# benmcclusky/Residual-TD3-Robot-Navigation

Measured on AMD Instinct MI355X. Metric: env-steps/sec at 65 536 parallel envs (full residual-TD3 update), higher is better.
Workload: dtype f32-accurate MLP: fp16x2 split (22-bit operands) on fp16 MFMA, f32 accumulate; f32 edge layers / losses / Adam; fp64 env state; 1 GPU; config3: 65536 envs + residual-TD3 (2x256 MLPs); envs_per_gpu=65536, envs_per_group=1024, hidden=256, layers=2, batch=32768, rank_batch=32768, parallelism=independent-env-blocks x1

## Files before the change

### residual-td3-robot-navigation_amd/csrc/learner_kernels.hip

```cpp
#include "mlp_common.h"

namespace {

struct WgradArgs {
    MlpDev net[2];
    int64_t M;
    const float* in;
    int ld_in, in_col;
    const float* acts[2];
    const float* dz[2];
    const float* dy[2];
    int ld_dy;
    const uint16_t* masks[2];
    float* slabs[2];
    int splits;
    int tk;
    int TT;
    int tn;
    int TN;
    int n_hid;
    int fact;
    int64_t per_split;
    int64_t per_wave;
    int64_t skew;
};

#ifdef NAV_WGRAD_TRACE
__device__ unsigned long long g_wgrad_trace[2][4][8][8];
#define WG_MARK(kid, k)                                                                        \
    do {                                                                                       \
        const int b_ = blockIdx.x == 0 ? 0 : blockIdx.x == 1 ? 1 : blockIdx.x == 128 ? 2         \
                       : blockIdx.x == 255 ? 3 : -1;                                           \
        if (b_ >= 0 && (threadIdx.x & 63) == 0)                                                \
            g_wgrad_trace[kid][b_][threadIdx.x >> 6][k] = __builtin_readcyclecounter();         \
    } while (0)
#else
#define WG_MARK(kid, k) \
    do {                \
    } while (0)
#endif

constexpr int WG_WAVES = 8;
#ifndef NAV_WG_SKEW_FACT
#define NAV_WG_SKEW_FACT 64
#endif
#ifndef NAV_WG_SKEW_OPND
#define NAV_WG_SKEW_OPND 128
#endif
constexpr int WG_TOTAL = 256;
constexpr int WG_THREADS = WG_WAVES * 64;
constexpr int WG_TILE = 64;
constexpr int WG_CHUNK = 64;
constexpr int WG_STAGE_FLOATS = WG_CHUNK * 6;
inline size_t wgrad_lds_bytes() {
    return ((size_t)WG_WAVES * WG_TILE * WG_TILE + (size_t)WG_WAVES * 2 * WG_STAGE_FLOATS) * 4;
}
__host__ __device__ inline bool wgrad_fact_ok(int hp, int n_hidden) {
    return n_hidden == 2 && hp % WG_TILE == 0;
}
struct WgradTiling {
    int tn, tk, TN, TT, jobs;
};
inline WgradTiling wgrad_tiling(int d_out, int hp, int n_hidden) {
    WgradTiling t;
    const bool f1 = wgrad_fact_ok(hp, n_hidden) && d_out == 1;
    const bool wide = f1 && hp % 256 == 0;
    t.tn = wide ? 256 : f1 && hp % 128 == 0 ? 128 : WG_TILE;
    t.tk = wide ? 32 : WG_TILE;
    t.TN = (hp + t.tn - 1) / t.tn;
    t.TT = (hp + t.tk - 1) / t.tk;
    t.jobs = (n_hidden > 1 ? n_hidden - 1 : 0) * t.TN * t.TT;
    return t;
}

template <bool PR, bool QR, bool RA_ = false>
NAV_DEV void wgrad_rows(const WgradArgs& a, int y, int L, int n0, int k0, int64_t r_lo,
                        int64_t r_hi, float* stage, f32x16 (&acc)[2][2]) {
    const MlpDev& net = a.net[y];
    const int hp = net.hp, nh = net.n_hidden, d_in = net.d_in, d_out = net.d_out;
    const int lane = threadIdx.x & 63, h = lane >> 5, l32 = lane & 31;
    const int64_t M = a.M, MH = M * hp;
    const bool nv1 = n0 + 32 < hp, kv1 = k0 + 32 < hp;
    const int cn[2] = {n0 + l32, nv1 ? n0 + 32 + l32 : n0 + l32};
    const int ck[2] = {k0 + l32, kv1 ? k0 + 32 + l32 : k0 + l32};
    float wo[2][2] = {{0.f, 0.f}, {0.f, 0.f}}, w0[2][4] = {}, b0[2] = {0.f, 0.f};
    if (PR) {
        const float* Wo = net.params + net.w_off[nh];
#pragma unroll
        for (int i = 0; i < 2; ++i) {
            wo[i][0] = Wo[cn[i]];
            wo[i][1] = d_out > 1 ? Wo[hp + cn[i]] : 0.f;
        }
    }
    if (QR) {
        const float* W0 = net.params + net.w_off[0];
        const float* bb = net.params + net.b_off[0];
#pragma unroll
        for (int j = 0; j < 2; ++j) {
#pragma unroll
            for (int k = 0; k < 4; ++k) w0[j][k] = k < d_in ? W0[ck[j] * d_in + k] : 0.f;
            b0[j] = bb[ck[j]];
        }
    }
    constexpr bool RA = RA_ && (PR != QR);
    constexpr int HS = WG_CHUNK / 8;
    const int NTm = hp >> 5;
// ... 67 lines not shown
            if ((!RA || s % HS == 0) && rb + 2 * s >= r_hi) break;
            if constexpr (RA) {
                if (s % HS == 0) window(s);
            }
            const int rr = 2 * s + h;
            float p[2], q[2];
            if (PR) {
                const float2 g = *reinterpret_cast<const float2*>(gs + rr * 2);
                const int sh = 16 * ((s >> 1) & 1) + 2 * (s & 1) + 4 * ((s & 15) >> 2);
#pragma unroll
                for (int i = 0; i < 2; ++i) {
                    const uint32_t bit = (mw[i][s >> 4] >> sh) & 1u;
                    p[i] = bit ? top_unit(g.x, g.y, wo[i][0], wo[i][1]) : 0.f;
                }
            } else if constexpr (RA) {
#pragma unroll
                for (int i = 0; i < 2; ++i) p[i] = ps[RA && !PR ? s % HS : 0][i];
            } else {
                const int64_t r = rb + rr;
                const bool ok = r < r_hi;
                const float* src = Psv + (ok ? r : r_lo) * hp;
#pragma unroll
                for (int i = 0; i < 2; ++i) p[i] = ok ? src[cn[i]] : 0.f;
            }
            if (QR) {
                const float4 x = *reinterpret_cast<const float4*>(xs + rr * 4);
#pragma unroll
                for (int j = 0; j < 2; ++j) q[j] = layer0_unit(x, w0[j][0], w0[j][1], w0[j][2], w0[j][3], b0[j]);
            } else if constexpr (RA) {
#pragma unroll
                for (int j = 0; j < 2; ++j) q[j] = qs[RA && !QR ? s % HS : 0][j];
            } else {
                const int64_t r = rb + rr;
                const bool ok = r < r_hi;
                const float* src = Qsv + (ok ? r : r_lo) * hp;
#pragma unroll
                for (int j = 0; j < 2; ++j) q[j] = ok ? src[ck[j]] : 0.f;
            }
            acc[0][0] = mfma(p[0], q[0], acc[0][0]);
            if (kv1) acc[0][1] = mfma(p[0], q[1], acc[0][1]);
            if (nv1) acc[1][0] = mfma(p[1], q[0], acc[1][0]);
            if (nv1 && kv1) acc[1][1] = mfma(p[1], q[1], acc[1][1]);
        }
        if (more) {
            park();
#pragma unroll
            for (int i = 0; i < 2; ++i)
#pragma unroll
                for (int t = 0; t < 2; ++t) mw[i][t] = cm[i][t] >> h;
        }
    }
}

NAV_DEV void row_maxima(const WgradArgs& a, int y, int64_t r_lo, int64_t r_hi, float (&G)[2],
                        float (&X)[4]) {
    const int lane = threadIdx.x & 63, d_in = a.net[y].d_in, d_out = a.net[y].d_out;
    float g0 = 0.f, g1 = 0.f, x0 = 0.f, x1 = 0.f, x2 = 0.f, x3 = 0.f;
    constexpr int RU = 4;
    const float* xin = a.in + a.in_col;
    const bool xv4 = d_in == 4 && (a.ld_in & 3) == 0 && ((uintptr_t)xin & 15) == 0;
    const bool xv2 = d_in == 2 && (a.ld_in & 1) == 0 && ((uintptr_t)xin & 7) == 0;
    const bool gv2 = d_out == 2 && (a.ld_dy & 1) == 0 && ((uintptr_t)a.dy[y] & 7) == 0;
    for (int64_t rb = r_lo; rb < r_hi; rb += 64 * RU) {
        float gv[RU][2], xv[RU][4];
#pragma unroll
        for (int u = 0; u < RU; ++u) {
            gv[u][0] = gv[u][1] = 0.f;
            xv[u][0] = xv[u][1] = xv[u][2] = xv[u][3] = 0.f;
            if (rb + 64 * u >= r_hi) continue;
            const int64_t r = rb + 64 * u + lane;
            if (r >= r_hi) continue;
            const float* g = a.dy[y] + r * a.ld_dy;
            const float* x = xin + r * a.ld_in;
            if (gv2) {
                const float2 v = *reinterpret_cast<const float2*>(g);
                gv[u][0] = v.x;
                gv[u][1] = v.y;
            } else {
                gv[u][0] = g[0];
                if (d_out > 1) gv[u][1] = g[1];
            }
            if (xv4) {
                const float4 v = *reinterpret_cast<const float4*>(x);
                xv[u][0] = v.x; xv[u][1] = v.y; xv[u][2] = v.z; xv[u][3] = v.w;
            } else if (xv2) {
                const float2 v = *reinterpret_cast<const float2*>(x);
                xv[u][0] = v.x; xv[u][1] = v.y;
            } else {
#pragma unroll
                for (int i = 0; i < 4; ++i)
                    if (d_in > i) xv[u][i] = x[i];
            }
        }
#pragma unroll
        for (int u = 0; u < RU; ++u) {
            g0 = fmaxf(g0, fabsf(gv[u][0]));
            g1 = fmaxf(g1, fabsf(gv[u][1]));
            x0 = fmaxf(x0, fabsf(xv[u][0]));
            x1 = fmaxf(x1, fabsf(xv[u][1]));
            x2 = fmaxf(x2, fabsf(xv[u][2]));
            x3 = fmaxf(x3, fabsf(xv[u][3]));
        }
    }
    auto su = [](float v) { return __int_as_float(__builtin_amdgcn_readfirstlane(__float_as_int(wave_max_abs(v)))); };
    G[0] = su(g0);
    G[1] = su(g1);
    X[0] = su(x0);
    X[1] = su(x1);
    X[2] = su(x2);
    X[3] = su(x3);
}

NAV_DEV float h0_bound(const float (&X)[4], float wa, float wb, float bias) {
    const int h = (threadIdx.x & 63) >> 5;
    const float part = (h ? X[1] : X[0]) * fabsf(wa) + (h ? X[3] : X[2]) * fabsf(wb) + fabsf(bias);
    return part + __shfl_xor(part, 32, 64);
}

NAV_DEV int cap_exp_finite(int e, float m) {
    if (!(m > 0.f)) return e;
    int E;
    (void)frexpf(m, &E);
    return min(e, 126 - E);
}

NAV_DEV void wgrad_rows_mfma(const WgradArgs& a, int y, int n0, int k0, int64_t r_lo,
                             int64_t r_hi, f32x16 (&acc)[2][2]) {
    const MlpDev& net = a.net[y];
    const int hp = net.hp, nh = net.n_hidden, d_in = net.d_in, d_out = net.d_out;
    const int lane = threadIdx.x & 63, h = lane >> 5, l32 = lane & 31;
    const int64_t M = a.M;
    const int NTm = hp >> 5;
    float wob[2], w0b[2][2], bob[2];
    {
        const float* Wo = net.params + net.w_off[nh];
        const float* W0 = net.params + net.w_off[0];
        const float* bb = net.params + net.b_off[0];
#pragma unroll
        for (int i = 0; i < 2; ++i) {
            wob[i] = h < d_out ? Wo[h * hp + n0 + 32 * i + l32] : 0.f;
            const int c = k0 + 32 * i + l32;
            w0b[i][0] = h < d_in ? W0[c * d_in + h] : 0.f;
            w0b[i][1] = 2 + h < d_in ? W0[c * d_in + 2 + h] : 0.f;
            bob[i] = h == 0 ? bb[c] : 0.f;
        }
    }
    if (r_lo >= r_hi) return;
    const uint16_t* mk = a.masks[y] + (size_t)(nh - 1) * mask_rowtiles(M) * NTm * 64 +
                         (size_t)(n0 >> 5) * 64 + lane;
    const size_t mstride = (size_t)NTm * 64;
    const float* dyp = a.dy[y];
    const int ld_dy = a.ld_dy, ld_in = a.ld_in;
    const float* xin = a.in + a.in_col;
    const int gk = h < d_out ? h : 0, xk0 = h < d_in ? h : 0, xk1 = 2 + h < d_in ? 2 + h : 0;
    struct Raw {
        float g, x0, x1;
        uint32_t m0, m1;
    };
    const float* gp = dyp + (r_lo + l32) * ld_dy + gk;
    const float* xp = xin + (r_lo + l32) * ld_in;
    const uint16_t* mp = mk + (size_t)(r_lo >> 5) * mstride;
    const int64_t gstep = 32 * (int64_t)ld_dy, xstep = 32 * (int64_t)ld_in;
    int64_t rl = r_lo;
    auto load = [&](int64_t) {
        Raw v;
        if (rl + 32 <= r_hi) {
            v.g = *gp;
            v.x0 = xp[xk0];
            v.x1 = xp[xk1];
            v.m0 = mp[0];
            v.m1 = mp[64];
        } else {
            const bool ok = rl + l32 < r_hi;
            const float* g = ok ? gp : dyp + r_lo * ld_dy + gk;
            const float* x = ok ? xp : xin + r_lo * ld_in;
            v.g = *g;
            v.x0 = x[xk0];
            v.x1 = x[xk1];
            v.m0 = mp[0];
            v.m1 = mp[64];
        }
        gp += gstep;
        xp += xstep;
        mp += mstride;
        rl += 32;
        return v;
    };
    float bc[2];
    const bool x23 = d_in > 2;
    auto issue = [&](int64_t rt, const Raw& v, f32x16 (&P)[2], f32x16 (&Q)[2]) {
        const bool ok = rt + l32 < r_hi && h < d_out;
        const float g = ok ? v.g : 0.f;
        const float x0 = h < d_in ? v.x0 : 0.f, x1 = 2 + h < d_in ? v.x1 : 0.f;
        const f32x16 zero = {};
#pragma unroll
        for (int i = 0; i < 2; ++i) {
            P[i] = mfma(g, wob[i], zero);
            f32x16 b;
#pragma unroll
            for (int e = 0; e < 16; ++e) b[e] = bc[i];
            Q[i] = mfma(x0, w0b[i][0], b);
        }
        if (x23) {
#pragma unroll
            for (int i = 0; i < 2; ++i) Q[i] = mfma(x1, w0b[i][1], Q[i]);
        }
    };
    auto finish = [&](const Raw& v, f32x16 (&P)[2], f32x16 (&Q)[2]) {
#pragma unroll
        for (int e = 0; e < 16; ++e) {
            P[0][e] = __int_as_float(__float_as_int(P[0][e]) & __builtin_amdgcn_sbfe((int)v.m0, e, 1));
            P[1][e] = __int_as_float(__float_as_int(P[1][e]) & __builtin_amdgcn_sbfe((int)v.m1, e, 1));
            Q[0][e] = __int_as_float(max(__float_as_int(Q[0][e]), 0));
            Q[1][e] = __int_as_float(max(__float_as_int(Q[1][e]), 0));
        }
    };
    Raw cur = load(r_lo);
    Raw nxt = cur;
    if (r_lo + 32 < r_hi) nxt = load(r_lo + 32);
    int ep[2], eq[2];
    {
        float G[2], X[4];
        WG_MARK(1, 2);
        row_maxima(a, y, r_lo, r_hi, G, X);
        WG_MARK(1, 3);
#pragma unroll
        for (int i = 0; i < 2; ++i) {
            float b = G[h] * fabsf(wob[i]);
            b += __shfl_xor(b, 32, 64);
#pragma unroll
            for (int m = 1; m < 32; m <<= 1) b = fmaxf(b, __shfl_xor(b, m, 64));
            ep[i] = pow2_exp(b);
            wob[i] = ldexpf(wob[i], ep[i]);
            float wm = fmaxf(fmaxf(fabsf(w0b[i][0]), fabsf(w0b[i][1])), fabsf(bob[i]));
            wm = fmaxf(wm, __shfl_xor(wm, 32, 64));
            eq[i] = cap_exp_finite(pow2_exp(h0_bound(X, w0b[i][0], w0b[i][1], bob[i])), wm);
            w0b[i][0] = ldexpf(w0b[i][0], eq[i]);
            w0b[i][1] = ldexpf(w0b[i][1], eq[i]);
            bob[i] = ldexpf(bob[i], eq[i]);
            bc[i] = bob[i] + __shfl_xor(bob[i], 32, 64);
        }
    }
    for (int64_t rt = r_lo; rt < r_hi; rt += 32) {
        Raw nn = nxt;
        if (rt + 64 < r_hi) nn = load(rt + 64);
        f32x16 P[2], Q[2];
        issue(rt, cur, P, Q);
        finish(cur, P, Q);
#pragma unroll
        for (int s2 = 0; s2 < 2; ++s2) {
            Split2 sp[2], sq[2];
#pragma unroll
            for (int i = 0; i < 2; ++i) {
                float vp[8], vq[8];
#pragma unroll
                for (int t = 0; t < 8; ++t) {
                    vp[t] = P[i][8 * s2 + t];
                    vq[t] = Q[i][8 * s2 + t];
                }
                sp[i] = split2_8(vp);
                sq[i] = split2_8(vq);
            }
#pragma unroll
            for (int i = 0; i < 2; ++i)
#pragma unroll
                for (int j = 0; j < 2; ++j) acc[i][j] = mfma_x3s(sp[i], sq[j], acc[i][j]);
        }
        cur = nxt;
        nxt = nn;
    }
    WG_MARK(1, 4);
#pragma unroll
    for (int i = 0; i < 2; ++i)
#pragma unroll
        for (int j = 0; j < 2; ++j)
#pragma unroll
            for (int e = 0; e < 16; ++e) acc[i][j][e] = ldexpf(acc[i][j][e], -(ep[i] + eq[j]));
}



template <int NI, int D, int KH, bool GV, bool XV>
NAV_DEV void wgrad_rows_fact(const WgradArgs& a, int y, int n0, int k0, int64_t r_lo,
                             int64_t r_hi, const char* tab, f32x16 (&out)[NI][KH]) {
    const MlpDev& net = a.net[y];
    const int hp = net.hp, d_in = net.d_in;
    const int lane = threadIdx.x & 63, h = lane >> 5, l32 = lane & 31;
    const int64_t M = a.M;
    const int NTm = hp >> 5;
    f32x16 acc[D][NI][KH];
#pragma unroll
    for (int d = 0; d < D; ++d)
#pragma unroll
        for (int i = 0; i < NI; ++i)
#pragma unroll
            for (int j = 0; j < KH; ++j)
#pragma unroll
                for (int e = 0; e < 16; ++e) acc[d][i][j][e] = 0.f;
    float w0b[KH][2], bob[KH];
    {
        const float* W0 = net.params + net.w_off[0];
        const float* bb = net.params + net.b_off[0];
#pragma unroll
        for (int j = 0; j < KH; ++j) {
            const int c = k0 + 32 * j + l32;
            w0b[j][0] = h < d_in ? W0[c * d_in + h] : 0.f;
            w0b[j][1] = 2 + h < d_in ? W0[c * d_in + 2 + h] : 0.f;
            bob[j] = h == 0 ? bb[c] : 0.f;
        }
    }
    int eh[KH], eg[D];
    float sg[D];
    float bcj[KH];
    const bool x23 = d_in > 2;
    const size_t mstride = (size_t)NTm * 64;
    const uint16_t* mp = a.masks[y] + (size_t)mask_rowtiles(M) * mstride +
                         (size_t)(n0 >> 5) * 64 + lane + (size_t)(r_lo >> 5) * mstride;
    const float* dyp = a.dy[y];
    const int ld_dy = a.ld_dy, ld_in = a.ld_in;
    const int xk0 = h < d_in ? h : 0, xk1 = 2 + h < d_in ? 2 + h : 0;
    constexpr bool MP = NI == 8;
    constexpr int NM = MP ? NI / 2 : NI;
    struct Raw {
        float x0, x1;
        uint32_t m[NM];
    };
    auto load_masks = [&](const uint16_t* m, Raw& v) {
#pragma unroll
        for (int u = 0; u < NM; ++u)
            v.m[u] = MP ? (uint32_t)m[2 * u * 64] | ((uint32_t)m[(2 * u + 1) * 64] << 16)
                        : (uint32_t)m[u * 64];
    };
    const bool xrow4 = d_in == 4 && (ld_in & 3) == 0 && (((uintptr_t)(a.in + a.in_col)) & 15) == 0;
    auto load_raw = [&](int64_t rt, Raw& v) {
        const int64_t rx = rt + l32 < r_hi ? rt + l32 : r_lo;
        const float* x = a.in + a.in_col + rx * ld_in;
        if (xrow4) {
            const float4 u = *reinterpret_cast<const float4*>(x);
            v.x0 = h ? u.y : u.x;
            v.x1 = h ? u.w : u.z;
        } else {
            v.x0 = x[xk0];
            v.x1 = x[xk1];
        }
        load_masks(mp + (size_t)((rt - r_lo) >> 5) * mstride, v);
    };
    auto tile = [&](const Raw& cur, const float (&gs)[2][D][8]) {
        const float x0 = h < d_in ? cur.x0 : 0.f, x1 = 2 + h < d_in ? cur.x1 : 0.f;
#pragma unroll
        for (int j = 0; j < KH; ++j) {
            f32x16 Z;
#pragma unroll
            for (int e = 0; e < 16; ++e) Z[e] = bcj[j];
            Z = mfma(x0, w0b[j][0], Z);
            if (x23) Z = mfma(x1, w0b[j][1], Z);
#pragma unroll
            for (int s2 = 0; s2 < 2; ++s2)
#pragma unroll
                for (int d = 0; d < D; ++d) {
                    float q[8];
#pragma unroll
                    for (int t = 0; t < 8; ++t)
                        q[t] = __int_as_float(max(__float_as_int(Z[8 * s2 + t]), 0)) * gs[s2][d][t];
                    const Split2 sq = split2_8(q);
#pragma unroll
                    for (int i = 0; i < NI; ++i) {
                        uint32_t ta = MP ? ((cur.m[i >> 1] >> (16 * (i & 1) + 8 * s2)) & 0xFFu) << 4
                                         : (s2 == 0 ? cur.m[i] << 4 : cur.m[i] >> 4) & 0xFF0u;
                        asm volatile("" : "+v"(ta));
                        const f16x8 pi = *reinterpret_cast<const f16x8*>(tab + ta);
                        acc[d][i][j] = mfma_h(pi, sq.l, acc[d][i][j]);
// ... 13 lines not shown
                const float* g = gp + (16 * s2 + 8 * qq) * ldg;
                if (GV && D == 1) {
                    const float4 u = *reinterpret_cast<const float4*>(g);
                    gs[s2][0][4 * qq] = u.x; gs[s2][0][4 * qq + 1] = u.y;
                    gs[s2][0][4 * qq + 2] = u.z; gs[s2][0][4 * qq + 3] = u.w;
                } else if (GV) {
                    const float4 u0 = *reinterpret_cast<const float4*>(g);
                    const float4 u1 = *reinterpret_cast<const float4*>(g + 4);
                    gs[s2][0][4 * qq] = u0.x; gs[s2][D - 1][4 * qq] = u0.y;
                    gs[s2][0][4 * qq + 1] = u0.z; gs[s2][D - 1][4 * qq + 1] = u0.w;
                    gs[s2][0][4 * qq + 2] = u1.x; gs[s2][D - 1][4 * qq + 2] = u1.y;
                    gs[s2][0][4 * qq + 3] = u1.z; gs[s2][D - 1][4 * qq + 3] = u1.w;
                } else {
#pragma unroll
                    for (int t = 0; t < 4; ++t)
#pragma unroll
                        for (int d = 0; d < D; ++d) gs[s2][d][4 * qq + t] = g[t * ldg + d];
                }
            }
    };
    auto scale_g = [&](float (&gs)[2][D][8]) {
        if (D == 1) return;
#pragma unroll
        for (int s2 = 0; s2 < 2; ++s2)
#pragma unroll
            for (int d = 0; d < D; ++d)
#pragma unroll
                for (int t = 0; t < 8; ++t) gs[s2][d][t] *= sg[d];
    };
    constexpr bool GPF = D == 1;
    const int64_t nfull = (r_full - r_lo) >> 5;
    const float* xq = a.in + a.in_col + (r_lo + l32) * (int64_t)ld_in;
    const uint16_t* mq = mp;
    const float* gq = dyp + (r_lo + 4 * h) * (int64_t)ldg;
    const int64_t xstep = 32 * (int64_t)ld_in, gstep = 32 * (int64_t)ldg;
    auto load_full = [&](Raw& v, float (&gs)[2][D][8]) {
        if (XV) {
            const float4 u = *reinterpret_cast<const float4*>(xq);
            v.x0 = h ? u.y : u.x;
            v.x1 = h ? u.w : u.z;
        } else {
            v.x0 = xq[xk0];
            v.x1 = xq[xk1];
        }
        load_masks(mq, v);
        if (GPF) load_g_at(gq, gs);
        xq += xstep;
        mq += mstride;
        gq += gstep;
    };
    Raw c0, c1;
    float g0[2][D][8], g1[2][D][8];
    if (nfull > 0) load_full(c0, g0);
    {
        float G[2], X[4];
        WG_MARK(0, 2);
        row_maxima(a, y, r_lo, r_hi, G, X);
        WG_MARK(0, 3);
#pragma unroll
        for (int d = 0; d < D; ++d) {
            eg[d] = pow2_exp_to(G[d], 8);
            sg[d] = D == 1 ? 1.f : ldexpf(1.f, eg[d]);
        }
#pragma unroll
        for (int j = 0; j < KH; ++j) {
            eh[j] = __builtin_amdgcn_readfirstlane(
                pow2_exp_to(wave_max_abs(h0_bound(X, w0b[j][0], w0b[j][1], bob[j])), 7));
            if (D == 1) eh[j] = min(max(eh[j] + eg[0], -126), 120);
            eh[j] = __builtin_amdgcn_readfirstlane(cap_exp_finite(
                eh[j], wave_max_abs(fmaxf(fmaxf(fabsf(w0b[j][0]), fabsf(w0b[j][1])),
                                          fabsf(bob[j])))));
            w0b[j][0] = ldexpf(w0b[j][0], eh[j]);
            w0b[j][1] = ldexpf(w0b[j][1], eh[j]);
            bob[j] = ldexpf(bob[j], eh[j]);
            bcj[j] = bob[j] + __shfl_xor(bob[j], 32, 64);
        }
        if (D == 1) eg[0] = 0;
    }
    for (int64_t t = 0; t < nfull; ++t) {
        if (t + 1 < nfull) load_full(c1, g1);
        if (!GPF) load_g_at(dyp + (r_lo + 32 * t + 4 * h) * (int64_t)ldg, g0);
        scale_g(g0);
        tile(c0, g0);
        c0 = c1;
        if (GPF) {
#pragma unroll
            for (int s2 = 0; s2 < 2; ++s2)
#pragma unroll
                for (int d = 0; d < D; ++d)
#pragma unroll
                    for (int e = 0; e < 8; ++e) g0[s2][d][e] = g1[s2][d][e];
        }
    }
    WG_MARK(0, 4);
    if (r_full < r_hi) {
        Raw cur;
        load_raw(r_full, cur);
        float gs[2][D][8];
#pragma unroll
        for (int e = 0; e < 16; ++e) {
            const int64_t r = r_full + acc_row(e, h);
#pragma unroll
            for (int d = 0; d < D; ++d) gs[e >> 3][d][e & 7] = r < r_hi ? dyp[r * ld_dy + d] * sg[d] : 0.f;
        }
        tile(cur, gs);
    }
    const float* Wo = net.params + net.w_off[net.n_hidden];
#pragma unroll
    for (int i = 0; i < NI; ++i) {
        if (NI == 8 && i > 0 && i % 2 == 0) __builtin_amdgcn_sched_barrier(0);
#pragma unroll
        for (int q = 0; q < 4; ++q) {
            const int n = n0 + 32 * i + 8 * q + 4 * h;
            float4 wv[D];
#pragma unroll
            for (int d = 0; d < D; ++d) {
                const float* w = Wo + d * hp + n;
                wv[d] = make_float4(w[0], w[1], w[2], w[3]);
            }
#pragma unroll
            for (int t = 0; t < 4; ++t) {
                const int e = 4 * q + t;
#pragma unroll
                for (int j = 0; j < KH; ++j) {
                    const float w0 = (t == 0 ? wv[0].x : t == 1 ? wv[0].y : t == 2 ? wv[0].z : wv[0].w) * 0.5f;
                    float v = w0 * ldexpf(acc[0][i][j][e], -(eh[j] + eg[0]));
                    if (D > 1) {
                        const float w1 = (t == 0 ? wv[D - 1].x : t == 1 ? wv[D - 1].y
                                          : t == 2 ? wv[D - 1].z : wv[D - 1].w) * 0.5f;
                        v = fmaf(w1, ldexpf(acc[D - 1][i][j][e], -(eh[j] + eg[D - 1])), v);
                    }
                    out[i][j][e] = v;
                }
            }
        }
    }
}

template <int NI, int KH>
NAV_DEV void wgrad_reduce_write(const WgradArgs& a, int y, int split, int L, int n0, int k0,
                                const f32x16 (&acc)[NI][KH], float* red) {
    constexpr int T = NI * 32 * 32 * KH;
    constexpr int R = (WG_WAVES * WG_TILE * WG_TILE) / T < WG_WAVES
                          ? (WG_WAVES * WG_TILE * WG_TILE) / T : WG_WAVES;
    const MlpDev& net = a.net[y];
    const int hp = net.hp;
    const int wv = wave_id(), lane = threadIdx.x & 63, h = lane >> 5, l32 = lane & 31;
    const int rot = (lane >> 2) & 3;
    float4* mine = reinterpret_cast<float4*>(red + (wv % R) * T);
#pragma unroll
    for (int round = 0; round < WG_WAVES / R; ++round) {
        if (wv / R == round) {
#pragma unroll
            for (int i = 0; i < NI; ++i)
#pragma unroll
                for (int j = 0; j < KH; ++j) {
                    float4* p = mine + ((i * KH + j) * 64 + lane) * 4;
#pragma unroll
                    for (int c = 0; c < 4; ++c) {
                        float4 v = make_float4(acc[i][j][4 * c], acc[i][j][4 * c + 1],
                                               acc[i][j][4 * c + 2], acc[i][j][4 * c + 3]);
                        if (round) {
                            const float4 o = p[c ^ rot];
                            v = make_float4(o.x + v.x, o.y + v.y, o.z + v.z, o.w + v.w);
                        }
                        p[c ^ rot] = v;
                    }
                }
        }
        __syncthreads();
    }
    float* o = a.slabs[y] + (int64_t)split * hidden_w_count(net) + (int64_t)(L - 1) * hp * hp;
// ... 4 lines not shown
#pragma unroll
        for (int w = 0; w < R; ++w) {
            const float4* p = slots + (size_t)w * (T / 4) + (b * 64 + lane) * 4;
#pragma unroll
            for (int c = 0; c < 4; ++c) {
                const float4 u = p[c ^ rot];
                if (w == 0) {
                    v[4 * c] = u.x; v[4 * c + 1] = u.y; v[4 * c + 2] = u.z; v[4 * c + 3] = u.w;
                } else {
                    v[4 * c] += u.x; v[4 * c + 1] += u.y; v[4 * c + 2] += u.z; v[4 * c + 3] += u.w;
                }
            }
        }
        const int col = k0 + 32 * j + l32;
#pragma unroll
        for (int e = 0; e < 16; ++e) {
            const int n = n0 + 32 * i + acc_row(e, h);
            if (n < hp && col < hp) o[(int64_t)n * hp + col] = v[e];
        }
    }
}

struct TileJob {
    int y, job, split, L, n0, k0;
};
NAV_DEV TileJob wgrad_job(const WgradArgs& a, int b, int total) {
    const int v = (total % 8 == 0) ? (b % 8) * (total / 8) + b / 8 : b;
    const int grp = v / a.n_hid, TT = a.TT, TN = a.TN;
    TileJob t;
    t.job = v % a.n_hid;
    t.y = grp / a.splits;
    t.split = grp % a.splits;
    t.L = t.job / (TN * TT) + 1;
    t.n0 = ((t.job % (TN * TT)) / TT) * a.tn;
    t.k0 = (t.job % TT) * a.tk;
    return t;
}

NAV_DEV void wave_rows(const WgradArgs& a, int split, int wv, int64_t skew, int64_t& r_lo,
                       int64_t& r_hi) {
    const int64_t M = a.M;
    const int64_t s_lo = (int64_t)split * a.per_split < M ? (int64_t)split * a.per_split : M;
    const int64_t s_hi = s_lo + a.per_split < M ? s_lo + a.per_split : M;
    const int64_t pa = a.per_wave + skew, pb = a.per_wave - skew;
    const int64_t off = wv < WG_WAVES / 2 ? wv * pa : (WG_WAVES / 2) * pa + (wv - WG_WAVES / 2) * pb;
    const int64_t len = wv < WG_WAVES / 2 ? pa : pb;
    r_lo = s_lo + off < s_hi ? s_lo + off : s_hi;
    r_hi = r_lo + len < s_hi ? r_lo + len : s_hi;
}

template <int NI, int D, int KH>
NAV_DEV void wgrad_tile_fact(const WgradArgs& a, const TileJob& t, float* smem, uint4* tab) {
    WG_MARK(0, 0);
    if (threadIdx.x < 256) {
        const uint32_t b = threadIdx.x;
        uint32_t w[4];
#pragma unroll
        for (int d = 0; d < 4; ++d)
            w[d] = ((b >> (2 * d)) & 1u ? 0x4000u : 0u) | ((b >> (2 * d + 1)) & 1u ? 0x40000000u : 0u);
        tab[b] = make_uint4(w[0], w[1], w[2], w[3]);
    }
    __syncthreads();
    WG_MARK(0, 1);
    int64_t r_lo, r_hi;
    wave_rows(a, t.split, wave_id(), a.skew, r_lo, r_hi);
    f32x16 out[NI][KH];
    const char* tb = reinterpret_cast<const char*>(tab);
    const bool gv = a.ld_dy == D && ((uintptr_t)a.dy[t.y] & 15) == 0;
    const bool xv = a.net[t.y].d_in == 4 && (a.ld_in & 3) == 0 &&
                    ((uintptr_t)(a.in + a.in_col) & 15) == 0;
    if (gv && xv) wgrad_rows_fact<NI, D, KH, true, true>(a, t.y, t.n0, t.k0, r_lo, r_hi, tb, out);
    else if (gv) wgrad_rows_fact<NI, D, KH, true, false>(a, t.y, t.n0, t.k0, r_lo, r_hi, tb, out);
    else if (xv) wgrad_rows_fact<NI, D, KH, false, true>(a, t.y, t.n0, t.k0, r_lo, r_hi, tb, out);
    else wgrad_rows_fact<NI, D, KH, false, false>(a, t.y, t.n0, t.k0, r_lo, r_hi, tb, out);
    WG_MARK(0, 5);
    wgrad_reduce_write<NI, KH>(a, t.y, t.split, t.L, t.n0, t.k0, out, smem);
    WG_MARK(0, 6);
}

template <bool GEN>
NAV_DEV void wgrad_tile(const WgradArgs& a, const TileJob& t, float* smem) {
    WG_MARK(1, 0);
    const int y = t.y, split = t.split, L = t.L, n0 = t.n0, k0 = t.k0;
    const int nh = a.net[y].n_hidden;
    const int wv = wave_id();
    const bool pr = L == nh - 1, qr = L == 1;
    const bool full = n0 + WG_TILE <= a.net[y].hp && k0 + WG_TILE <= a.net[y].hp;
    const bool opnd = pr && qr && full;
    int64_t r_lo, r_hi;
    wave_rows(a, split, wv, opnd ? a.skew : 0, r_lo, r_hi);
    float* red = smem;
    float* stage = smem + WG_WAVES * WG_TILE * WG_TILE + wv * 2 * WG_STAGE_FLOATS;
    f32x16 acc[2][2];
#pragma unroll
    for (int i = 0; i < 2; ++i)
#pragma unroll
        for (int j = 0; j < 2; ++j)
#pragma unroll
            for (int e = 0; e < 16; ++e) acc[i][j][e] = 0.f;
    if constexpr (GEN) {
        if (pr && qr) wgrad_rows<true, true, true>(a, y, L, n0, k0, r_lo, r_hi, stage, acc);
        else if (pr) wgrad_rows<true, false, true>(a, y, L, n0, k0, r_lo, r_hi, stage, acc);
        else if (qr) wgrad_rows<false, true, true>(a, y, L, n0, k0, r_lo, r_hi, stage, acc);
        else wgrad_rows<false, false, true>(a, y, L, n0, k0, r_lo, r_hi, stage, acc);
    } else {
        if (opnd) wgrad_rows_mfma(a, y, n0, k0, r_lo, r_hi, acc);
        else if (pr && qr) wgrad_rows<true, true>(a, y, L, n0, k0, r_lo, r_hi, stage, acc);
        else if (pr) wgrad_rows<true, false>(a, y, L, n0, k0, r_lo, r_hi, stage, acc);
        else if (qr) wgrad_rows<false, true>(a, y, L, n0, k0, r_lo, r_hi, stage, acc);
        else wgrad_rows<false, false>(a, y, L, n0, k0, r_lo, r_hi, stage, acc);
    }
    WG_MARK(1, 5);
    wgrad_reduce_write<2, 2>(a, y, split, L, n0, k0, acc, red);
    WG_MARK(1, 6);
}

#ifndef NAV_LEARNER_POP
__global__ __launch_bounds__(WG_THREADS) void k_wgrad(WgradArgs a) {
    extern __shared__ __attribute__((aligned(16))) float smem[];
    wgrad_tile<false>(a, wgrad_job(a, blockIdx.x, gridDim.x), smem);
}
__global__ __launch_bounds__(WG_THREADS) void k_wgrad_gen(WgradArgs a) {
    extern __shared__ __attribute__((aligned(16))) float smem[];
    wgrad_tile<true>(a, wgrad_job(a, blockIdx.x, gridDim.x), smem);
}
template <int NI, int D, int KH>
__global__ __launch_bounds__(WG_THREADS) void k_wgrad_fact(WgradArgs a) {
    extern __shared__ __attribute__((aligned(16))) float smem[];
    __shared__ uint4 tab[256];
    wgrad_tile_fact<NI, D, KH>(a, wgrad_job(a, blockIdx.x, gridDim.x), smem, tab);
}
#endif

struct PackInfo {
    int hp, n_hidden, d_out;
    int64_t w_off[kMaxLayers];
    float* packed;
};

struct PackJob {
    const float* p;
    PackInfo pk;
};
struct PackArgs {
    PackJob j[8];
    int n, per_net, cg;
};

#ifndef NAV_LEARNER_POP
__global__ __launch_bounds__(kBlock) void k_pack_img(PackArgs a) {
#include "pack_img_body.inc"
}
#endif

NAV_DEV float adam1(float& p, float g, float& m, float& v, float b1w, float b2, float omb2,
                    float eps, float step_size, float bc2s) {
    m = fmaf(b1w, g - m, m);
    v = v * b2 + (omb2 * g) * g;
    const float denom = sqrtf(v) / bc2s + eps;
    p = p + (-step_size) * (m / denom);
    return p;
}

struct PolyPair {
    float4* t;
    const float4* s;
    int64_t n4;
};
struct PolyArgs {
    PolyPair q[4];
    int n;
    int64_t total4;
    float omt, tau;
};

struct RedNet {
    MlpDev net;
    const float4* hs;
    const float4* es;
    float4* grad;
    float4* p;
    float4* m;
// ... 715 lines not shown
    NAV_CHECK_LAUNCH();
    return 0;
}

int nav_fill(float* x, int64_t n, float value, void* stream) {
    if (n < 0 || (n && !x)) return NAV_EINVAL;
    if (n == 0) return 0;
    hipLaunchKernelGGL(k_fill, dim3(blocks_for(n)), dim3(kBlock), 0, S(stream), x, n, value);
    NAV_CHECK_LAUNCH();
    return 0;
}

int nav_strided_copy(const float* src, int32_t ld_src, int32_t col_src, float* dst,
                     int32_t ld_dst, int32_t col_dst, int64_t rows, int32_t cols, void* stream) {
    if (rows < 0 || cols < 0 || (rows && cols && (!src || !dst))) return NAV_EINVAL;
    if (rows == 0 || cols == 0) return 0;
    hipLaunchKernelGGL(k_strided_copy, dim3(blocks_for(rows * cols)), dim3(kBlock), 0, S(stream),
                       src, ld_src, col_src, dst, ld_dst, col_dst, rows, cols);
    NAV_CHECK_LAUNCH();
    return 0;
}

#endif

}

#if defined(NAV_WGRAD_TRACE) && !defined(NAV_LEARNER_POP)
extern "C" int nav_wgrad_trace_read(unsigned long long* host, int n) {
    const size_t bytes = sizeof(g_wgrad_trace);
    if (!host || (size_t)n * sizeof(unsigned long long) < bytes) return NAV_EINVAL;
    const hipError_t e = hipMemcpyFromSymbol(host, HIP_SYMBOL(g_wgrad_trace), bytes);
    return e == hipSuccess ? 0 : -(int)e;
}
#endif

#ifdef NAV_LEARNER_POP
namespace {

constexpr int kMaxMembers = 256;

struct LearnMember {
    WgradArgs wg[2];
    RedArgs red[3];
    PackArgs pack[3];
    double lr[2];
};
static_assert(sizeof(LearnMember) % 4 == 0, "copied as 32-bit words");

template <bool GEN>
__global__ __launch_bounds__(WG_THREADS) void k_wgrad_pop(const LearnMember* __restrict__ tab,
                                                          int group) {
    extern __shared__ __attribute__((aligned(16))) float smem[];
    const WgradArgs& a = tab[blockIdx.y].wg[group];
    wgrad_tile<GEN>(a, wgrad_job(a, blockIdx.x, gridDim.x), smem);
}
template <int NI, int D, int KH>
__global__ __launch_bounds__(WG_THREADS) void k_wgrad_fact_pop(const LearnMember* __restrict__ tab,
                                                               int group) {
    extern __shared__ __attribute__((aligned(16))) float smem[];
    __shared__ uint4 ftab[256];
    const WgradArgs& a = tab[blockIdx.y].wg[group];
    wgrad_tile_fact<NI, D, KH>(a, wgrad_job(a, blockIdx.x, gridDim.x), smem, ftab);
}

__global__ __launch_bounds__(kBlock) void k_grad_reduce_adam_pop(
    const LearnMember* __restrict__ tab, int which, AdamStep st, double bc1) {
    const LearnMember& m = tab[blockIdx.y];
    st.step_size = (float)(m.lr[which ? 1 : 0] / bc1);
    grad_reduce_body<true, true>(m.red[which], st);
}

__global__ __launch_bounds__(kBlock) void k_pack_img_pop(const LearnMember* __restrict__ tab,
                                                         int set) {
    const PackArgs& a = tab[blockIdx.y].pack[set];
#include "pack_img_body.inc"
}

int learn_member_fill(const nav_td3_member& t, int64_t B, int32_t sc, int32_t sa, LearnMember& e,
                      int (&blocks)[3]) {
    if (B < 1 || sc < 1 || sa < 1 || !t.batch || !t.batch_actor || !t.da) return NAV_EINVAL;
    const int64_t nblk = nav_mlp_row_blocks(B);
    const nav_mlp crit[2] = {t.critics[0], t.critics[1]};
    const nav_mlp tcrit[2] = {t.target_critics[0], t.target_critics[1]};
    if (t.actor.n_hidden != t.critics[0].n_hidden || t.actor.d_in != 2 || t.actor.d_out != 2 ||
        crit[0].d_in != 4 || crit[0].d_out != 1 || crit[1].d_in != 4 || crit[1].d_out != 1)
        return NAV_EINVAL;
    if (t.actor.n_hidden > 1) {
        int rc = wgrad_args(crit, 2, B, t.batch, 8, 0, t.acts, t.dz, t.dq, 1, t.masks,
                            t.hidden_slabs, sc, e.wg[0]);
        if (rc) return rc;
        const float* acts_a[1] = {t.acts_actor};
        const float* dz_a[1] = {t.dz_actor};
        const float* dy_a[1] = {t.da};
        const uint16_t* mk_a[1] = {t.masks_actor};
        float* hs_a[1] = {t.hidden_slabs[0]};
        rc = wgrad_args(&t.actor, 1, B, t.batch_actor, 8, 0, acts_a, dz_a, dy_a, 2, mk_a, hs_a,
                        sa, e.wg[1]);
        if (rc) return rc;
    }
    const float zero[2] = {0.f, 0.f};
    PackSet ps[3];
    int rc = red_args(crit, 2, t.hidden_slabs, sc, t.edge_slabs, nblk, t.grad_critic, t.m_critic,
                      t.v_critic, 0.f, 0.f, 0.f, zero, zero, nullptr, nullptr, nullptr, 0, 0.f,
                      e.red[0], &blocks[0], &ps[0]);
    if (rc) return rc;
    const float* hs_a[1] = {t.hidden_slabs[0]};
    const float* es_a[1] = {t.edge_slabs_actor};
    float* g_a[1] = {t.grad_actor};
    float* m_a[1] = {t.m_actor};
    float* v_a[1] = {t.v_actor};
    rc = red_args(&t.actor, 1, hs_a, sa, es_a, nblk, g_a, m_a, v_a, 0.f, 0.f, 0.f, zero, zero,
                  nullptr, nullptr, nullptr, 0, 0.f, e.red[1], &blocks[1], &ps[1]);
    if (rc) return rc;
    rc = red_args(&t.actor, 1, hs_a, sa, es_a, nblk, g_a, m_a, v_a, 0.f, 0.f, 0.f, zero, zero,
// ... 135 lines not shown
```

Baseline: 164.8 million env-steps/s.

## Hoist wgrad prologue loads ahead of LDS table build and maxima pass

```diff
diff --git a/residual-td3-robot-navigation_amd/csrc/learner_kernels.hip b/residual-td3-robot-navigation_amd/csrc/learner_kernels.hip
--- a/residual-td3-robot-navigation_amd/csrc/learner_kernels.hip
+++ b/residual-td3-robot-navigation_amd/csrc/learner_kernels.hip
@@ -25,14 +25,51 @@
     int64_t skew;
 };
 
+struct WgNet {
+    const float* params;
+    const float* dy;
+    const uint16_t* masks;
+    int64_t w0, b0, wo;
+    int hp, d_in, d_out;
+};
+NAV_DEV void wg_touch_args(const WgradArgs& a) {
+    const uint32_t* p = reinterpret_cast<const uint32_t*>(&a);
+    constexpr int n = (int)(sizeof(WgradArgs) / 4);
+    uint32_t v[(n + 15) / 16 + 1];
+#pragma unroll
+    for (int i = 0; i < (n + 15) / 16; ++i) v[i] = p[16 * i];
+    v[(n + 15) / 16] = p[n - 1];
+#pragma unroll
+    for (int i = 0; i <= (n + 15) / 16; ++i) asm volatile("" ::"s"(v[i]));
+}
+NAV_DEV WgNet wg_net(const WgradArgs& a, int y) {
+    const WgNet n0 = {a.net[0].params, a.dy[0], a.masks[0], a.net[0].w_off[0], a.net[0].b_off[0],
+                      a.net[0].w_off[2], a.net[0].hp, a.net[0].d_in, a.net[0].d_out};
+    const WgNet n1 = {a.net[1].params, a.dy[1], a.masks[1], a.net[1].w_off[0], a.net[1].b_off[0],
+                      a.net[1].w_off[2], a.net[1].hp, a.net[1].d_in, a.net[1].d_out};
+    WgNet n;
+    n.params = y ? n1.params : n0.params;
+    n.dy = y ? n1.dy : n0.dy;
+    n.masks = y ? n1.masks : n0.masks;
+    n.w0 = y ? n1.w0 : n0.w0;
+    n.b0 = y ? n1.b0 : n0.b0;
+    n.wo = y ? n1.wo : n0.wo;
+    n.hp = y ? n1.hp : n0.hp;
+    n.d_in = y ? n1.d_in : n0.d_in;
+    n.d_out = y ? n1.d_out : n0.d_out;
+    return n;
+}
+
 #ifdef NAV_WGRAD_TRACE
-__device__ unsigned long long g_wgrad_trace[2][4][8][8];
+__device__ unsigned long long g_wgrad_trace[2][4][8][16];
 #define WG_MARK(kid, k)                                                                        \
     do {                                                                                       \
+        asm volatile("" ::: "memory");                                                         \
         const int b_ = blockIdx.x == 0 ? 0 : blockIdx.x == 1 ? 1 : blockIdx.x == 128 ? 2         \
                        : blockIdx.x == 255 ? 3 : -1;                                           \
         if (b_ >= 0 && (threadIdx.x & 63) == 0)                                                \
             g_wgrad_trace[kid][b_][threadIdx.x >> 6][k] = __builtin_readcyclecounter();         \
+        asm volatile("" ::: "memory");                                                         \
     } while (0)
 #else
 #define WG_MARK(kid, k) \
@@ -52,6 +89,7 @@
 constexpr int WG_TILE = 64;
 constexpr int WG_CHUNK = 64;
 constexpr int WG_STAGE_FLOATS = WG_CHUNK * 6;
+constexpr int WG_FACT_TAB = 256, WG_FACT_LDS = WG_FACT_TAB + 2 * 256 / 4;
 inline size_t wgrad_lds_bytes() {
     return ((size_t)WG_WAVES * WG_TILE * WG_TILE + (size_t)WG_WAVES * 2 * WG_STAGE_FLOATS) * 4;
 }
@@ -225,55 +263,94 @@
     }
 }
 
-NAV_DEV void row_maxima(const WgradArgs& a, int y, int64_t r_lo, int64_t r_hi, float (&G)[2],
-                        float (&X)[4]) {
-    const int lane = threadIdx.x & 63, d_in = a.net[y].d_in, d_out = a.net[y].d_out;
-    float g0 = 0.f, g1 = 0.f, x0 = 0.f, x1 = 0.f, x2 = 0.f, x3 = 0.f;
-    constexpr int RU = 4;
+constexpr int WG_MAXU = 6;
+struct MaxRows {
+    float g[WG_MAXU][2], x[WG_MAXU][4];
+};
+NAV_DEV void maxima_load(const WgradArgs& a, const WgNet& net, int64_t rb, int64_t r_hi,
+                         MaxRows& v) {
+    const int lane = threadIdx.x & 63, d_in = net.d_in, d_out = net.d_out;
     const float* xin = a.in + a.in_col;
     const bool xv4 = d_in == 4 && (a.ld_in & 3) == 0 && ((uintptr_t)xin & 15) == 0;
     const bool xv2 = d_in == 2 && (a.ld_in & 1) == 0 && ((uintptr_t)xin & 7) == 0;
-    const bool gv2 = d_out == 2 && (a.ld_dy & 1) == 0 && ((uintptr_t)a.dy[y] & 7) == 0;
-    for (int64_t rb = r_lo; rb < r_hi; rb += 64 * RU) {
-        float gv[RU][2], xv[RU][4];
-#pragma unroll
-        for (int u = 0; u < RU; ++u) {
-            gv[u][0] = gv[u][1] = 0.f;
-            xv[u][0] = xv[u][1] = xv[u][2] = xv[u][3] = 0.f;
-            if (rb + 64 * u >= r_hi) continue;
-            const int64_t r = rb + 64 * u + lane;
-            if (r >= r_hi) continue;
-            const float* g = a.dy[y] + r * a.ld_dy;
-            const float* x = xin + r * a.ld_in;
-            if (gv2) {
-                const float2 v = *reinterpret_cast<const float2*>(g);
-                gv[u][0] = v.x;
-                gv[u][1] = v.y;
-            } else {
-                gv[u][0] = g[0];
-                if (d_out > 1) gv[u][1] = g[1];
+    const bool gv2 = d_out == 2 && (a.ld_dy & 1) == 0 && ((uintptr_t)net.dy & 7) == 0;
+#pragma unroll
+    for (int u = 0; u < WG_MAXU; ++u) {
+        v.g[u][0] = v.g[u][1] = 0.f;
+        v.x[u][0] = v.x[u][1] = v.x[u][2] = v.x[u][3] = 0.f;
+    }
+    if (rb >= r_hi) return;
+    const float* g[WG_MAXU];
+    const float* x[WG_MAXU];
+#pragma unroll
+    for (int u = 0; u < WG_MAXU; ++u) {
+        const int64_t r = rb + 64 * u + lane, rc = r < r_hi ? r : rb;
+        g[u] = net.dy + rc * a.ld_dy;
+        x[u] = xin + rc * a.ld_in;
+    }
+#define WG_UOK(u) (rb + 64 * (u) < r_hi)
+    if (xv4) {
+#pragma unroll
+        for (int u = 0; u < WG_MAXU; ++u)
+            if (WG_UOK(u)) {
+                const float4 w = *reinterpret_cast<const float4*>(x[u]);
+                v.x[u][0] = w.x; v.x[u][1] = w.y; v.x[u][2] = w.z; v.x[u][3] = w.w;
             }
-            if (xv4) {
-                const float4 v = *reinterpret_cast<const float4*>(x);
-                xv[u][0] = v.x; xv[u][1] = v.y; xv[u][2] = v.z; xv[u][3] = v.w;
-            } else if (xv2) {
-                const float2 v = *reinterpret_cast<const float2*>(x);
-                xv[u][0] = v.x; xv[u][1] = v.y;
-            } else {
-#pragma unroll
-                for (int i = 0; i < 4; ++i)
-                    if (d_in > i) xv[u][i] = x[i];
+    } else if (xv2) {
+#pragma unroll
+        for (int u = 0; u < WG_MAXU; ++u)
+            if (WG_UOK(u)) {
+                const float2 w = *reinterpret_cast<const float2*>(x[u]);
+                v.x[u][0] = w.x; v.x[u][1] = w.y;
             }
-        }
-#pragma unroll
-        for (int u = 0; u < RU; ++u) {
-            g0 = fmaxf(g0, fabsf(gv[u][0]));
-            g1 = fmaxf(g1, fabsf(gv[u][1]));
-            x0 = fmaxf(x0, fabsf(xv[u][0]));
-            x1 = fmaxf(x1, fabsf(xv[u][1]));
-            x2 = fmaxf(x2, fabsf(xv[u][2]));
-            x3 = fmaxf(x3, fabsf(xv[u][3]));
-        }
+    } else {
+#pragma unroll
+        for (int i = 0; i < 4; ++i)
+            if (d_in > i) {
+#pragma unroll
+                for (int u = 0; u < WG_MAXU; ++u)
+                    if (WG_UOK(u)) v.x[u][i] = x[u][i];
+            }
+    }
+    if (gv2) {
+#pragma unroll
+        for (int u = 0; u < WG_MAXU; ++u)
+            if (WG_UOK(u)) {
+                const float2 w = *reinterpret_cast<const float2*>(g[u]);
+                v.g[u][0] = w.x;
+                v.g[u][1] = w.y;
+            }
+    } else {
+#pragma unroll
+        for (int u = 0; u < WG_MAXU; ++u)
+            if (WG_UOK(u)) v.g[u][0] = g[u][0];
+        if (d_out > 1) {
+#pragma unroll
+            for (int u = 0; u < WG_MAXU; ++u)
+                if (WG_UOK(u)) v.g[u][1] = g[u][1];
+        }
+    }
+#undef WG_UOK
+}
+NAV_DEV void row_maxima(const WgradArgs& a, const WgNet& net, int64_t r_lo, int64_t r_hi,
+                        const MaxRows& first, float (&G)[2], float (&X)[4]) {
+    float g0 = 0.f, g1 = 0.f, x0 = 0.f, x1 = 0.f, x2 = 0.f, x3 = 0.f;
+    auto fold = [&](const MaxRows& v) {
+#pragma unroll
+        for (int u = 0; u < WG_MAXU; ++u) {
+            g0 = fmaxf(g0, fabsf(v.g[u][0]));
+            g1 = fmaxf(g1, fabsf(v.g[u][1]));
+            x0 = fmaxf(x0, fabsf(v.x[u][0]));
+            x1 = fmaxf(x1, fabsf(v.x[u][1]));
+            x2 = fmaxf(x2, fabsf(v.x[u][2]));
+            x3 = fmaxf(x3, fabsf(v.x[u][3]));
+        }
+    };
+    fold(first);
+    for (int64_t rb = r_lo + 64 * WG_MAXU; rb < r_hi; rb += 64 * WG_MAXU) {
+        MaxRows v;
+        maxima_load(a, net, rb, r_hi, v);
+        fold(v);
     }
     auto su = [](float v) { return __int_as_float(__builtin_amdgcn_readfirstlane(__float_as_int(wave_max_abs(v)))); };
     G[0] = su(g0);
@@ -299,30 +376,49 @@
 
 NAV_DEV void wgrad_rows_mfma(const WgradArgs& a, int y, int n0, int k0, int64_t r_lo,
                              int64_t r_hi, f32x16 (&acc)[2][2]) {
-    const MlpDev& net = a.net[y];
-    const int hp = net.hp, nh = net.n_hidden, d_in = net.d_in, d_out = net.d_out;
+    const WgNet net = wg_net(a, y);
+    MaxRows mrows;
+    maxima_load(a, net, r_lo, r_hi, mrows);
+    WG_MARK(1, 11);
+    constexpr int nh = 2;
+    const int hp = net.hp, d_in = net.d_in, d_out = net.d_out;
     const int lane = threadIdx.x & 63, h = lane >> 5, l32 = lane & 31;
     const int64_t M = a.M;
     const int NTm = hp >> 5;
     float wob[2], w0b[2][2], bob[2];
     {
-        const float* Wo = net.params + net.w_off[nh];
-        const float* W0 = net.params + net.w_off[0];
-        const float* bb = net.params + net.b_off[0];
+        const float* Wo = net.params + net.wo;
+        const float* W0 = net.params + net.w0;
+        const float* bb = net.params + net.b0;
+        const int ho = h < d_out ? h : 0, h0 = h < d_in ? h : 0, h2 = 2 + h < d_in ? 2 + h : 0;
 #pragma unroll
         for (int i = 0; i < 2; ++i) {
-            wob[i] = h < d_out ? Wo[h * hp + n0 + 32 * i + l32] : 0.f;
             const int c = k0 + 32 * i + l32;
-            w0b[i][0] = h < d_in ? W0[c * d_in + h] : 0.f;
-            w0b[i][1] = 2 + h < d_in ? W0[c * d_in + 2 + h] : 0.f;
-            bob[i] = h == 0 ? bb[c] : 0.f;
-        }
-    }
-    if (r_lo >= r_hi) return;
-    const uint16_t* mk = a.masks[y] + (size_t)(nh - 1) * mask_rowtiles(M) * NTm * 64 +
+            const float vo = Wo[ho * hp + n0 + 32 * i + l32], va = W0[c * d_in + h0],
+                        vb = W0[c * d_in + h2], vc = bb[c];
+            wob[i] = h < d_out ? vo : 0.f;
+            w0b[i][0] = h < d_in ? va : 0.f;
+            w0b[i][1] = 2 + h < d_in ? vb : 0.f;
+            bob[i] = h == 0 ? vc : 0.f;
+        }
+    }
+    WG_MARK(1, 9);
+    auto zero_acc = [&]() {
+#pragma unroll
+        for (int i = 0; i < 2; ++i)
+#pragma unroll
+            for (int j = 0; j < 2; ++j)
+#pragma unroll
+                for (int e = 0; e < 16; ++e) acc[i][j][e] = 0.f;
+    };
+    if (r_lo >= r_hi) {
+        zero_acc();
+        return;
+    }
+    const uint16_t* mk = net.masks + (size_t)(nh - 1) * mask_rowtiles(M) * NTm * 64 +
                          (size_t)(n0 >> 5) * 64 + lane;
     const size_t mstride = (size_t)NTm * 64;
-    const float* dyp = a.dy[y];
+    const float* dyp = net.dy;
     const int ld_dy = a.ld_dy, ld_in = a.ld_in;
     const float* xin = a.in + a.in_col;
     const int gk = h < d_out ? h : 0, xk0 = h < d_in ? h : 0, xk1 = 2 + h < d_in ? 2 + h : 0;
@@ -395,7 +491,7 @@
     {
         float G[2], X[4];
         WG_MARK(1, 2);
-        row_maxima(a, y, r_lo, r_hi, G, X);
+        row_maxima(a, net, r_lo, r_hi, mrows, G, X);
         WG_MARK(1, 3);
 #pragma unroll
         for (int i = 0; i < 2; ++i) {
@@ -414,6 +510,9 @@
             bc[i] = bob[i] + __shfl_xor(bob[i], 32, 64);
         }
     }
+    WG_MARK(1, 10);
+    zero_acc();
+    WG_MARK(1, 8);
     for (int64_t rt = r_lo; rt < r_hi; rt += 32) {
         Raw nn = nxt;
         if (rt + 64 < r_hi) nn = load(rt + 64);
@@ -454,42 +553,43 @@
 
 
 template <int NI, int D, int KH, bool GV, bool XV>
-NAV_DEV void wgrad_rows_fact(const WgradArgs& a, int y, int n0, int k0, int64_t r_lo,
-                             int64_t r_hi, const char* tab, f32x16 (&out)[NI][KH]) {
-    const MlpDev& net = a.net[y];
+NAV_DEV void wgrad_rows_fact(const WgradArgs& a, const WgNet& net, int n0, int k0, int64_t r_lo,
+                             int64_t r_hi, uint4* lds_tab, f32x16 (&out)[NI][KH]) {
     const int hp = net.hp, d_in = net.d_in;
     const int lane = threadIdx.x & 63, h = lane >> 5, l32 = lane & 31;
     const int64_t M = a.M;
     const int NTm = hp >> 5;
+    const char* tab = reinterpret_cast<const char*>(lds_tab);
+    float* wos = reinterpret_cast<float*>(lds_tab + WG_FACT_TAB);
+    float wo_mine = 0.f;
+    if ((int)threadIdx.x < D * hp) wo_mine = (net.params + net.wo)[threadIdx.x];
+    MaxRows mrows;
+    maxima_load(a, net, r_lo, r_hi, mrows);
+    WG_MARK(0, 11);
     f32x16 acc[D][NI][KH];
-#pragma unroll
-    for (int d = 0; d < D; ++d)
-#pragma unroll
-        for (int i = 0; i < NI; ++i)
-#pragma unroll
-            for (int j = 0; j < KH; ++j)
-#pragma unroll
-                for (int e = 0; e < 16; ++e) acc[d][i][j][e] = 0.f;
     float w0b[KH][2], bob[KH];
     {
-        const float* W0 = net.params + net.w_off[0];
-        const float* bb = net.params + net.b_off[0];
+        const float* W0 = net.params + net.w0;
+        const float* bb = net.params + net.b0;
+        const int h0 = h < d_in ? h : 0, h2 = 2 + h < d_in ? 2 + h : 0;
 #pragma unroll
         for (int j = 0; j < KH; ++j) {
             const int c = k0 + 32 * j + l32;
-            w0b[j][0] = h < d_in ? W0[c * d_in + h] : 0.f;
-            w0b[j][1] = 2 + h < d_in ? W0[c * d_in + 2 + h] : 0.f;
-            bob[j] = h == 0 ? bb[c] : 0.f;
-        }
-    }
+            const float va = W0[c * d_in + h0], vb = W0[c * d_in + h2], vc = bb[c];
+            w0b[j][0] = h < d_in ? va : 0.f;
+            w0b[j][1] = 2 + h < d_in ? vb : 0.f;
+            bob[j] = h == 0 ? vc : 0.f;
+        }
+    }
+    WG_MARK(0, 9);
     int eh[KH], eg[D];
     float sg[D];
     float bcj[KH];
     const bool x23 = d_in > 2;
     const size_t mstride = (size_t)NTm * 64;
-    const uint16_t* mp = a.masks[y] + (size_t)mask_rowtiles(M) * mstride +
+    const uint16_t* mp = net.masks + (size_t)mask_rowtiles(M) * mstride +
                          (size_t)(n0 >> 5) * 64 + lane + (size_t)(r_lo >> 5) * mstride;
-    const float* dyp = a.dy[y];
+    const float* dyp = net.dy;
     const int ld_dy = a.ld_dy, ld_in = a.ld_in;
     const int xk0 = h < d_in ? h : 0, xk1 = 2 + h < d_in ? 2 + h : 0;
     constexpr bool MP = NI == 8;
@@ -609,10 +709,21 @@
     Raw c0, c1;
     float g0[2][D][8], g1[2][D][8];
     if (nfull > 0) load_full(c0, g0);
+    WG_MARK(0, 2);
+    if (threadIdx.x < 256) {
+        const uint32_t b = threadIdx.x;
+        uint32_t w[4];
+#pragma unroll
+        for (int d = 0; d < 4; ++d)
+            w[d] = ((b >> (2 * d)) & 1u ? 0x4000u : 0u) | ((b >> (2 * d + 1)) & 1u ? 0x40000000u : 0u);
+        lds_tab[b] = make_uint4(w[0], w[1], w[2], w[3]);
+    }
+    if ((int)threadIdx.x < D * hp) wos[threadIdx.x] = wo_mine;
+    __syncthreads();
+    WG_MARK(0, 1);
     {
         float G[2], X[4];
-        WG_MARK(0, 2);
-        row_maxima(a, y, r_lo, r_hi, G, X);
+        row_maxima(a, net, r_lo, r_hi, mrows, G, X);
         WG_MARK(0, 3);
 #pragma unroll
         for (int d = 0; d < D; ++d) {
@@ -634,6 +745,16 @@
         }
         if (D == 1) eg[0] = 0;
     }
+    WG_MARK(0, 10);
+#pragma unroll
+    for (int d = 0; d < D; ++d)
+#pragma unroll
+        for (int i = 0; i < NI; ++i)
+#pragma unroll
+            for (int j = 0; j < KH; ++j)
+#pragma unroll
+                for (int e = 0; e < 16; ++e) acc[d][i][j][e] = 0.f;
+    WG_MARK(0, 8);
     for (int64_t t = 0; t < nfull; ++t) {
         if (t + 1 < nfull) load_full(c1, g1);
         if (!GPF) load_g_at(dyp + (r_lo + 32 * t + 4 * h) * (int64_t)ldg, g0);
@@ -662,7 +783,6 @@
         }
         tile(cur, gs);
     }
-    const float* Wo = net.params + net.w_off[net.n_hidden];
 #pragma unroll
     for (int i = 0; i < NI; ++i) {
         if (NI == 8 && i > 0 && i % 2 == 0) __builtin_amdgcn_sched_barrier(0);
@@ -671,10 +791,7 @@
             const int n = n0 + 32 * i + 8 * q + 4 * h;
             float4 wv[D];
 #pragma unroll
-            for (int d = 0; d < D; ++d) {
-                const float* w = Wo + d * hp + n;
-                wv[d] = make_float4(w[0], w[1], w[2], w[3]);
-            }
+            for (int d = 0; d < D; ++d) wv[d] = *reinterpret_cast<const float4*>(wos + d * hp + n);
 #pragma unroll
             for (int t = 0; t < 4; ++t) {
                 const int e = 4 * q + t;
@@ -785,27 +902,18 @@
 template <int NI, int D, int KH>
 NAV_DEV void wgrad_tile_fact(const WgradArgs& a, const TileJob& t, float* smem, uint4* tab) {
     WG_MARK(0, 0);
-    if (threadIdx.x < 256) {
-        const uint32_t b = threadIdx.x;
-        uint32_t w[4];
-#pragma unroll
-        for (int d = 0; d < 4; ++d)
-            w[d] = ((b >> (2 * d)) & 1u ? 0x4000u : 0u) | ((b >> (2 * d + 1)) & 1u ? 0x40000000u : 0u);
-        tab[b] = make_uint4(w[0], w[1], w[2], w[3]);
-    }
-    __syncthreads();
-    WG_MARK(0, 1);
+    const WgNet net = wg_net(a, t.y);
     int64_t r_lo, r_hi;
     wave_rows(a, t.split, wave_id(), a.skew, r_lo, r_hi);
+    WG_MARK(0, 7);
     f32x16 out[NI][KH];
-    const char* tb = reinterpret_cast<const char*>(tab);
-    const bool gv = a.ld_dy == D && ((uintptr_t)a.dy[t.y] & 15) == 0;
-    const bool xv = a.net[t.y].d_in == 4 && (a.ld_in & 3) == 0 &&
+    const bool gv = a.ld_dy == D && ((uintptr_t)net.dy & 15) == 0;
+    const bool xv = net.d_in == 4 && (a.ld_in & 3) == 0 &&
                     ((uintptr_t)(a.in + a.in_col) & 15) == 0;
-    if (gv && xv) wgrad_rows_fact<NI, D, KH, true, true>(a, t.y, t.n0, t.k0, r_lo, r_hi, tb, out);
-    else if (gv) wgrad_rows_fact<NI, D, KH, true, false>(a, t.y, t.n0, t.k0, r_lo, r_hi, tb, out);
-    else if (xv) wgrad_rows_fact<NI, D, KH, false, true>(a, t.y, t.n0, t.k0, r_lo, r_hi, tb, out);
-    else wgrad_rows_fact<NI, D, KH, false, false>(a, t.y, t.n0, t.k0, r_lo, r_hi, tb, out);
+    if (gv && xv) wgrad_rows_fact<NI, D, KH, true, true>(a, net, t.n0, t.k0, r_lo, r_hi, tab, out);
+    else if (gv) wgrad_rows_fact<NI, D, KH, true, false>(a, net, t.n0, t.k0, r_lo, r_hi, tab, out);
+    else if (xv) wgrad_rows_fact<NI, D, KH, false, true>(a, net, t.n0, t.k0, r_lo, r_hi, tab, out);
+    else wgrad_rows_fact<NI, D, KH, false, false>(a, net, t.n0, t.k0, r_lo, r_hi, tab, out);
     WG_MARK(0, 5);
     wgrad_reduce_write<NI, KH>(a, t.y, t.split, t.L, t.n0, t.k0, out, smem);
     WG_MARK(0, 6);
@@ -815,22 +923,25 @@
 NAV_DEV void wgrad_tile(const WgradArgs& a, const TileJob& t, float* smem) {
     WG_MARK(1, 0);
     const int y = t.y, split = t.split, L = t.L, n0 = t.n0, k0 = t.k0;
-    const int nh = a.net[y].n_hidden;
+    const int nh = a.net[0].n_hidden, hp = a.net[0].hp;
     const int wv = wave_id();
     const bool pr = L == nh - 1, qr = L == 1;
-    const bool full = n0 + WG_TILE <= a.net[y].hp && k0 + WG_TILE <= a.net[y].hp;
+    const bool full = n0 + WG_TILE <= hp && k0 + WG_TILE <= hp;
     const bool opnd = pr && qr && full;
     int64_t r_lo, r_hi;
     wave_rows(a, split, wv, opnd ? a.skew : 0, r_lo, r_hi);
+    WG_MARK(1, 7);
     float* red = smem;
     float* stage = smem + WG_WAVES * WG_TILE * WG_TILE + wv * 2 * WG_STAGE_FLOATS;
     f32x16 acc[2][2];
-#pragma unroll
-    for (int i = 0; i < 2; ++i)
-#pragma unroll
-        for (int j = 0; j < 2; ++j)
-#pragma unroll
-            for (int e = 0; e < 16; ++e) acc[i][j][e] = 0.f;
+    if (GEN || !opnd) {
+#pragma unroll
+        for (int i = 0; i < 2; ++i)
+#pragma unroll
+            for (int j = 0; j < 2; ++j)
+#pragma unroll
+                for (int e = 0; e < 16; ++e) acc[i][j][e] = 0.f;
+    }
     if constexpr (GEN) {
         if (pr && qr) wgrad_rows<true, true, true>(a, y, L, n0, k0, r_lo, r_hi, stage, acc);
         else if (pr) wgrad_rows<true, false, true>(a, y, L, n0, k0, r_lo, r_hi, stage, acc);
@@ -851,6 +962,7 @@
 #ifndef NAV_LEARNER_POP
 __global__ __launch_bounds__(WG_THREADS) void k_wgrad(WgradArgs a) {
     extern __shared__ __attribute__((aligned(16))) float smem[];
+    wg_touch_args(a);
     wgrad_tile<false>(a, wgrad_job(a, blockIdx.x, gridDim.x), smem);
 }
 __global__ __launch_bounds__(WG_THREADS) void k_wgrad_gen(WgradArgs a) {
@@ -860,7 +972,8 @@
 template <int NI, int D, int KH>
 __global__ __launch_bounds__(WG_THREADS) void k_wgrad_fact(WgradArgs a) {
     extern __shared__ __attribute__((aligned(16))) float smem[];
-    __shared__ uint4 tab[256];
+    __shared__ uint4 tab[WG_FACT_LDS];
+    wg_touch_args(a);
     wgrad_tile_fact<NI, D, KH>(a, wgrad_job(a, blockIdx.x, gridDim.x), smem, tab);
 }
 #endif
@@ -1682,14 +1795,16 @@
                                                           int group) {
     extern __shared__ __attribute__((aligned(16))) float smem[];
     const WgradArgs& a = tab[blockIdx.y].wg[group];
+    if (!GEN) wg_touch_args(a);
     wgrad_tile<GEN>(a, wgrad_job(a, blockIdx.x, gridDim.x), smem);
 }
 template <int NI, int D, int KH>
 __global__ __launch_bounds__(WG_THREADS) void k_wgrad_fact_pop(const LearnMember* __restrict__ tab,
                                                                int group) {
     extern __shared__ __attribute__((aligned(16))) float smem[];
-    __shared__ uint4 ftab[256];
+    __shared__ uint4 ftab[WG_FACT_LDS];
     const WgradArgs& a = tab[blockIdx.y].wg[group];
+    wg_touch_args(a);
     wgrad_tile_fact<NI, D, KH>(a, wgrad_job(a, blockIdx.x, gridDim.x), smem, ftab);
 }
 
```

After: 166.3 million env-steps/s (median of 6 runs). No clear change (+0.9%).
